# balisujohn/tortoise.cpp

Hardware: AMD Instinct MI355X
Metric: audio-seconds/sec end-to-end (AR+diffusion+vocoder), 16 cands x 80 steps (higher is better)
Workload: dtype f16 MFMA inputs / f32 accumulate (diffusion, vocoder convs); f32 weights, f16 KV (AR)

## Files before the change

### tortoise.cpp_amd/csrc/gemm_f16.h

```cpp
#pragma once
#include <hip/hip_fp16.h>
#include <hip/hip_runtime.h>
#include <algorithm>
#include <cmath>
#include <cstdlib>
#include <type_traits>

namespace tts {

typedef _Float16 half8 __attribute__((ext_vector_type(8)));
typedef float floatx4 __attribute__((ext_vector_type(4)));

enum { GEMM_OUT_F32 = 0, GEMM_OUT_F16 = 1, GEMM_OUT_QKV = 2, GEMM_OUT_QKV_SPLIT = 3, GEMM_OUT_F32_SCALED = 4, GEMM_OUT_F32_STATS = 5, GEMM_OUT_F32_SCALED_STATS = 6 };
constexpr bool gemm_mode_qkv(int mode) { return mode == GEMM_OUT_QKV || mode == GEMM_OUT_QKV_SPLIT; }
constexpr bool gemm_mode_f32(int mode) { return mode == GEMM_OUT_F32 || mode == GEMM_OUT_F32_SCALED || mode == GEMM_OUT_F32_STATS || mode == GEMM_OUT_F32_SCALED_STATS; }
constexpr bool gemm_mode_scaled(int mode) { return mode == GEMM_OUT_F32_SCALED || mode == GEMM_OUT_F32_SCALED_STATS; }
constexpr bool gemm_mode_stats(int mode) { return mode == GEMM_OUT_F32_STATS || mode == GEMM_OUT_F32_SCALED_STATS; }

struct GemmArgs {
  const __half *A[3];
  int row_off[3];
  int nseg, kseg;
  int lda;
  const __half *W;
  int ldw_, w_off_[3], custom_w;
  const __half *Wf;
  int wreg;
  int M, N;
  const float *bias;
  const int *row_seq;
  float *outF; int ldo; const float *resid;
  __half *outH; int ldh;
  __half *outVt; int ldvt;
  __half *outH2, *outVt2;
  float alpha;
  long long *st_out;
  int st_stripe_ll;
  const int *chunk_seq;
  int dual_b;
  int mode;
  int th, cn;
  int ku;
};


__device__ __forceinline__ int lds_swz(int row) { return ((row >> 1) & 3) << 1; }
__device__ __forceinline__ int lds_off(int row, int chunk) { return row * 128 + ((chunk ^ lds_swz(row)) << 4); }

typedef const void __attribute__((address_space(1))) *gptr_t;
typedef void __attribute__((address_space(3))) *lptr_t;

__device__ __forceinline__ int vh_blk(int wm, int i) { return wm + 2 * i; }

__device__ __forceinline__ float split_lo(float x) { return x - __half2float(__float2half_rn(x)); }
__device__ __forceinline__ uint2 pack_half4(float a, float b, float c, float d) {
  const __half2 p0 = __floats2half2_rn(a, b), p1 = __floats2half2_rn(c, d);
  uint2 u;
  u.x = *(const unsigned *)&p0;
  u.y = *(const unsigned *)&p1;
  return u;
}

static constexpr int FX_STRIPES = 8;
__device__ __forceinline__ void fx_add(long long *dst, float p) {
  const float h = rintf(p * 256.0f);
  const float rem = p - h * (1.0f / 256.0f);
  atomicAdd((unsigned long long *)dst, (unsigned long long)(long long)h);
  atomicAdd((unsigned long long *)dst + 1, (unsigned long long)(long long)rintf(rem * 4503599627370496.0f));
}
__device__ __forceinline__ void fx_split(float p, long long &hi, long long &lo) {
  const float h = rintf(p * 256.0f);
  hi = (long long)h;
  lo = (long long)rintf((p - h * (1.0f / 256.0f)) * 4503599627370496.0f);
}
__host__ __device__ __forceinline__ double fx_value(long long hi, long long lo) { return (double)hi * (1.0 / 256.0) + (double)lo * (1.0 / 1152921504606846976.0); }
template <int CTRL> __device__ __forceinline__ float gemm_dpp(float x) {
  return __int_as_float(__builtin_amdgcn_update_dpp(0, __float_as_int(x), CTRL, 0xf, 0xf, false));
}
__device__ __forceinline__ float red_half_block(float x) {
  x += gemm_dpp<0xB1>(x);
  x += gemm_dpp<0x4E>(x);
  x += gemm_dpp<0x141>(x);
  auto a = __builtin_amdgcn_permlane32_swap(__float_as_uint(x), __float_as_uint(x), false, false);
  x = __uint_as_float(a[0]) + __uint_as_float(a[1]);
  auto b = __builtin_amdgcn_permlane16_swap(__float_as_uint(x), __float_as_uint(x), false, false);
  return __uint_as_float(b[0]) + __uint_as_float(b[1]);
}

enum { EPI_NO_RESID = 0, EPI_RESID_IN_ACC = 1, EPI_RESID_LOAD = 2 };
template <int MODE, int MI, int RESID>
__device__ __forceinline__ void gemm_epilogue_vh(const GemmArgs &g, floatx4 (&acc)[MI > 0 ? MI : 1][4], int m0, int n0, int wm, int wn, int fr, int fq) {
  constexpr int MA = MI > 0 ? MI : 1;
  if (MI == 0) return;
  if (gemm_mode_qkv(MODE)) {
    const int c0 = n0 + wn * 64, h = c0 / 192, w0 = c0 - h * 192;
    if (w0 >= 128) {
      const bool hb = g.bias != nullptr, hs = g.row_seq != nullptr;
      const float *bp = hb ? g.bias : (const float *)g.W;
      const int *sp = hs ? g.row_seq : (const int *)g.A[0];
      float bv[4];
      int4 sq[MA];
#pragma unroll
      for (int j = 0; j < 4; j++) bv[j] = bp[c0 + j * 16 + fr];
#pragma unroll
      for (int i = 0; i < MI; i++) sq[i] = *(const int4 *)(sp + m0 + vh_blk(wm, i) * 16 + fq * 4);
#pragma unroll
      for (int j = 0; j < 4; j++) bv[j] = hb ? bv[j] : 0.f;
#pragma unroll
      for (int i = 0; i < MI; i++) sq[i] = hs ? sq[i] : make_int4(0, 0, 0, 0);
#pragma unroll
      for (int i = 0; i < MI; i++) {
        const int rbase = m0 + vh_blk(wm, i) * 16 + fq * 4;
        const bool gd[4] = {sq[i].x < 0, sq[i].y < 0, sq[i].z < 0, sq[i].w < 0};
#pragma unroll
        for (int j = 0; j < 4; j++) {
          float v[4];
#pragma unroll
          for (int r = 0; r < 4; r++) v[r] = gd[r] ? 0.f : acc[i][j][r] + bv[j];
          *(uint2 *)(g.outVt + (size_t)(h * 64 + j * 16 + fr) * g.ldvt + rbase) = pack_half4(v[0], v[1], v[2], v[3]);
          if (MODE == GEMM_OUT_QKV_SPLIT)
            *(uint2 *)(g.outVt2 + (size_t)(h * 64 + j * 16 + fr) * g.ldvt + rbase) = pack_half4(split_lo(v[0]), split_lo(v[1]), split_lo(v[2]), split_lo(v[3]));
        }
      }
      return;
    }
  }
  const int col0 = n0 + wn * 64 + fq * 4;
  const bool hb = g.bias != nullptr, hs = g.row_seq != nullptr;
  const float *bp = hb ? g.bias : (const float *)g.W;
  const int *sp = hs ? g.row_seq : (const int *)g.A[0];
  float4 b4[4];
  int sq[MA];
  float4 rr[2][4];
  auto load_pair = [&](int p) {
#pragma unroll
    for (int q = 0; q < 2; q++) {
      const int i = min(2 * p + q, MI - 1);
      const float *rp = g.resid + (size_t)(m0 + vh_blk(wm, i) * 16 + fr) * g.ldo + col0;
#pragma unroll
      for (int j = 0; j < 4; j++) rr[q][j] = *(const float4 *)(rp + j * 16);
    }
  };
  if (RESID == EPI_RESID_LOAD) load_pair(0);
#pragma unroll
  for (int j = 0; j < 4; j++) b4[j] = *(const float4 *)(bp + col0 + j * 16);
#pragma unroll
  for (int i = 0; i < MI; i++) sq[i] = sp[m0 + vh_blk(wm, i) * 16 + fr];
#pragma unroll
  for (int j = 0; j < 4; j++) b4[j] = hb ? b4[j] : make_float4(0.f, 0.f, 0.f, 0.f);
#pragma unroll
  for (int i = 0; i < MI; i++) sq[i] = hs ? sq[i] : 0;
  auto finish = [&](int i, int j) {
    if (gemm_mode_scaled(MODE)) acc[i][j] *= g.alpha;
    float4 v = make_float4(acc[i][j][0] + b4[j].x, acc[i][j][1] + b4[j].y, acc[i][j][2] + b4[j].z, acc[i][j][3] + b4[j].w);
    if (sq[i] < 0) v = make_float4(0.f, 0.f, 0.f, 0.f);
    return v;
  };
  if (gemm_mode_f32(MODE)) {
    float ssum[MA][2], ssq[MA][2];
// ... 363 lines not shown
  int sq[MI];
#pragma unroll
  for (int j = 0; j < 2; j++) b4[j] = *(const float4 *)(bp + col0 + j * 16);
#pragma unroll
  for (int i = 0; i < MI; i++) sq[i] = sp[m0 + min(i, nblk - 1) * 16 + fr];
#pragma unroll
  for (int j = 0; j < 2; j++) b4[j] = hb ? b4[j] : make_float4(0.f, 0.f, 0.f, 0.f);
#pragma unroll
  for (int i = 0; i < MI; i++) sq[i] = hs ? sq[i] : 0;
  auto finish = [&](int i, int j) {
    float4 v = make_float4(acc[i][j][0] + b4[j].x, acc[i][j][1] + b4[j].y, acc[i][j][2] + b4[j].z, acc[i][j][3] + b4[j].w);
    if (sq[i] < 0) v = make_float4(0.f, 0.f, 0.f, 0.f);
    return v;
  };
  if (MODE == GEMM_OUT_F32) {
#pragma unroll
    for (int i = 0; i < MI; i++) {
      if (i < nblk) {
        float *op = g.outF + (size_t)(m0 + i * 16 + fr) * g.ldo + col0;
#pragma unroll
        for (int j = 0; j < 2; j++) *(float4 *)(op + j * 16) = finish(i, j);
      }
    }
  } else {
    const int h = c0 / 192, w0 = c0 - h * 192;
#pragma unroll
    for (int i = 0; i < MI; i++) {
      if (i < nblk) {
        __half *op = g.outH + (size_t)(m0 + i * 16 + fr) * g.ldh + h * 128 + w0 + fq * 4;
#pragma unroll
        for (int j = 0; j < 2; j++) {
          const float4 v = finish(i, j);
          *(uint2 *)(op + j * 16) = pack_half4(v.x, v.y, v.z, v.w);
          if (MODE == GEMM_OUT_QKV_SPLIT)
            *(uint2 *)(g.outH2 + (op - g.outH) + j * 16) = pack_half4(split_lo(v.x), split_lo(v.y), split_lo(v.z), split_lo(v.w));
        }
      }
    }
  }
}

template <int MODE, int MI, int D, bool NAT>
__device__ __forceinline__ void gemm_wreg_body(const GemmArgs &g, int m0, int n0, int nblk, int lane, int wave) {
  extern __shared__ __attribute__((aligned(16))) char smem_dyn[];
  char *smem = smem_dyn;
  constexpr int S = D + 1;
  constexpr int NPA = MI / 2;
  constexpr int PER = NPA + 4;
  static_assert(D == 1 || D == 2, "prefetch distance");
  const int T = g.kseg >> 6, KS = g.kseg >> 5;
  const int fr = lane & 15, fq = lane >> 4;
  unsigned aoff[NPA];
#pragma unroll
  for (int i = 0; i < NPA; i++) aoff[i] = (unsigned)(gemm_dma_off(wave + 4 * i, lane, 0, nblk * 16 - 1, g.lda) * 2);
  const char *aseg = (const char *)(g.A[0] + (ptrdiff_t)(g.row_off[0] + m0) * g.lda);
  const __half *wp0 = g.Wf + (size_t)((n0 >> 4) + wave * 2) * KS * 512, *wp1 = wp0 + (size_t)KS * 512;
  const unsigned wlane = lane * 16;
  const bool resid_first = MODE == GEMM_OUT_F32 && g.resid != nullptr;
  floatx4 acc[MI][2];
  gemm_acc_start<MODE, MI, 2>(g, acc, resid_first, n0 + wave * 32, fq, [&](int i) { return m0 + min(i, nblk - 1) * 16 + fr; });
  half8 w[S][2][2];
  auto issue = [&](int t, auto set_c) {
    constexpr int U = decltype(set_c)::value;
    const char *ab = aseg + (t << 7);
#pragma unroll
    for (int i = 0; i < NPA; i++) __builtin_amdgcn_global_load_lds((gptr_t)(ab + aoff[i]), (lptr_t)(smem + U * 16384 + (wave + 4 * i) * 1024), 16, 0, 0);
    const __half *q0 = wp0 + (size_t)t * 1024, *q1 = wp1 + (size_t)t * 1024;
    wreg_load<0>(w[U][0][0], q0, wlane);
    wreg_load<0>(w[U][0][1], q1, wlane);
    wreg_load<1024>(w[U][1][0], q0, wlane);
    wreg_load<1024>(w[U][1][1], q1, wlane);
  };
  auto kloop = [&]() {
    auto step = [&](int t, auto u_c) {
      constexpr int U = decltype(u_c)::value;
      if (D == 2 && t + 1 < T) wreg_wait<PER>(w[U][0][0], w[U][0][1], w[U][1][0], w[U][1][1]);
      else wreg_wait<0>(w[U][0][0], w[U][0][1], w[U][1][0], w[U][1][1]);
      asm volatile("s_waitcnt lgkmcnt(0)" ::: "memory");
      __builtin_amdgcn_s_barrier();
      if (t + D < T) issue(t + D, std::integral_constant<int, (U + D) % S>{});
      const char *sa = smem + U * 16384;
      constexpr int AHEAD = 2;
      half8 af[AHEAD + 1];
      auto frag = [&](int x) { return *(const half8 *)(sa + lds_off((x % MI) * 16 + fr, (x / MI) * 4 + fq)); };
#pragma unroll
      for (int x = 0; x < AHEAD; x++) af[x] = frag(x);
#pragma unroll
      for (int x = 0; x < 2 * MI; x++) {
        if (x + AHEAD < 2 * MI) af[(x + AHEAD) % (AHEAD + 1)] = frag(x + AHEAD);
        const int ks = x / MI, i = x % MI;
        const half8 a = af[x % (AHEAD + 1)];
#pragma unroll
        for (int j = 0; j < 2; j++) {
          if (NAT) acc[i][j] = __builtin_amdgcn_mfma_f32_16x16x32_f16(a, w[U][ks][j], acc[i][j], 0, 0, 0);
          else acc[i][j] = __builtin_amdgcn_mfma_f32_16x16x32_f16(w[U][ks][j], a, acc[i][j], 0, 0, 0);
        }
      }
      __builtin_amdgcn_sched_group_barrier(0x100, AHEAD, 0);
#pragma unroll
      for (int x = 0; x < 2 * MI; x++) {
        if (x + AHEAD < 2 * MI) __builtin_amdgcn_sched_group_barrier(0x100, 1, 0);
        __builtin_amdgcn_sched_group_barrier(0x008, 2, 0);
      }
    };
    for (int t0 = 0; t0 < T; t0 += S) {
      step(t0, std::integral_constant<int, 0>{});
      if (t0 + 1 < T) step(t0 + 1, std::integral_constant<int, 1>{});
      if (S == 3 && t0 + 2 < T) step(t0 + 2, std::integral_constant<int, S - 1>{});
    }
  };
  issue(0, std::integral_constant<int, 0>{});
  if (D == 2) issue(1, std::integral_constant<int, 1>{});
#pragma unroll
  for (int i = 0; i < MI; i++)
#pragma unroll
    for (int j = 0; j < 2; j++) asm volatile("" : "+v"(acc[i][j]));
  kloop();
  gemm_epilogue_wreg<MODE, MI, NAT>(g, acc, m0, n0, nblk, wave, fr, fq);
}

static constexpr int GEMM_WREG_D = 1, GEMM_WREG_LDS = (GEMM_WREG_D + 1) * 16384;
template <int MODE, int D = GEMM_WREG_D>
static __global__ __launch_bounds__(256, 4) void gemm_f16_wreg_kernel(GemmArgs g) {
  const int tid = threadIdx.x, lane = tid & 63, wave = __builtin_amdgcn_readfirstlane(tid >> 6);
  int m0, n0, nblk;
  if (!gemm_vh_tile(g, m0, n0, nblk)) return;
  if (gemm_mode_qkv(MODE) && ((n0 + wave * 32) % 192) >= 128) {
    if (nblk > 4) gemm_wreg_body<MODE, 8, D, true>(g, m0, n0, nblk, lane, wave);
    else gemm_wreg_body<MODE, 4, D, true>(g, m0, n0, nblk, lane, wave);
  } else {
    if (nblk > 4) gemm_wreg_body<MODE, 8, D, false>(g, m0, n0, nblk, lane, wave);
    else gemm_wreg_body<MODE, 4, D, false>(g, m0, n0, nblk, lane, wave);
  }
}
static inline bool gemm_takes_wreg(const GemmArgs &g, int th, int ku) {
  return g.wreg > 0 && g.Wf && g.nseg == 1 && !g.custom_w && th == 8 && ku == 1 && (g.kseg >> 6) >= 2 &&
         (g.mode == GEMM_OUT_F32 || g.mode == GEMM_OUT_QKV || g.mode == GEMM_OUT_QKV_SPLIT);
}

struct GemmGnPanelArgs {
  const __half *A; int lda;
  const __half *Wf;
  int N, K;
  const float *bias;
  const int *seq_start, *seq_len; int ns, rows_total;
  float eps; const float *gn_g, *gn_b, *ss; int do_silu, lut; __half *y; const int *seq_step; int ss_step_stride;
};
static constexpr int GEMM_GN_PANEL_ROWS = 896, GEMM_GN_PANEL_LDS = GEMM_GN_PANEL_ROWS * 128;
static constexpr int GEMM_GN_PANEL_WRING = 2 * 8192, GEMM_GN_PANEL_LDS_LAUNCH = GEMM_GN_PANEL_LDS + GEMM_GN_PANEL_WRING;
__device__ __forceinline__ int gnp_panel_f4(int t, int q) { return t * 128 + ((q ^ (t & 7)) << 4); }
template <int OFF> __device__ __forceinline__ void gnp_lds_read(half8 &d, unsigned addr) {
  asm volatile("ds_read_b128 %0, %1 offset:%2" : "=v"(d) : "v"(addr), "i"(OFF));
}
static inline int gemm_auto_th(int M, int N);
static inline bool gemm_gn_panel_takes(int option, bool stats, bool debug_sums, bool has_wf, int max_len, int rows, int N, int K) {
  return option != 0 && !stats && !debug_sums && has_wf && max_len >= 1 && max_len <= GEMM_GN_PANEL_ROWS && gemm_auto_th(rows, N) == 8 && (N % 64) == 0 && K >= 64 && (K % 64) == 0;
}
static inline int gemm_gn_panel_grid(int ns, int N) { return 8 * ((ns * (N >> 6) + 7) / 8); }

template <class TAIL>
static __global__ __launch_bounds__(512) void gemm_f16_gn_panel_kernel(GemmGnPanelArgs a, TAIL tail) {
  extern __shared__ __attribute__((aligned(16))) char smem_dyn[];
  char *smem = smem_dyn;
  const int tid = threadIdx.x, lane = tid & 63, wave = __builtin_amdgcn_readfirstlane(tid >> 6);
  const int np = a.N >> 6, nitems = a.ns * np, xcd = blockIdx.x & 7, idx = blockIdx.x >> 3;
  const int i0 = (int)((long long)nitems * xcd >> 3), i1 = (int)((long long)nitems * (xcd + 1) >> 3);
  if (idx >= i1 - i0) return;
  const int item = i0 + idx, s = item / np, n0 = (item - s * np) << 6;
  const int T = a.seq_len[s], r0 = a.seq_start[s];
  const int KT = a.K >> 6, fr = lane & 15, fq = lane >> 4;
  const int rb = wave * 112 + (lane >> 3), lda2 = a.lda * 2;
  const unsigned coloff = (unsigned)(((lane & 7) ^ lds_swz(lane >> 3)) << 4);
  const char *aseg = (const char *)(a.A + (size_t)r0 * a.lda);
  const size_t wstride = (size_t)(a.K >> 5) * 512;
  const __half *wsrc = a.Wf + (size_t)((n0 >> 4) + (wave & 3)) * wstride + (wave >> 2) * 512 + lane * 8;
  char *wring = smem + GEMM_GN_PANEL_LDS;
  const unsigned wfb = (unsigned)(size_t)(lptr_t)wring + lane * 16;
  const unsigned lds0 = (unsigned)(size_t)(lptr_t)smem + wave * 7 * 2048;
  const unsigned fb0 = lds0 + lds_off(fr, fq), fb1 = lds0 + lds_off(fr, 4 + fq);
  floatx4 acc[7][4];
#pragma unroll
  for (int i = 0; i < 7; i++)
#pragma unroll
    for (int j = 0; j < 4; j++) acc[i][j] = (floatx4){0.f, 0.f, 0.f, 0.f};
  auto dma = [&](int t) {
    const char *ab = aseg + (t << 7);
    int rbv = rb;
    asm volatile("" : "+v"(rbv));
#pragma unroll
    for (int i = 0; i < 14; i++) {
      const unsigned off = (unsigned)(min(rbv + 8 * i, T - 1) * lda2) + coloff;
      __builtin_amdgcn_global_load_lds((gptr_t)(ab + off), (lptr_t)(smem + (wave * 14 + i) * 1024), 16, 0, 0);
    }
  };
  auto wdma = [&](int t) { __builtin_amdgcn_global_load_lds((gptr_t)(wsrc + (size_t)t * 1024), (lptr_t)(wring + ((t & 1) << 13) + wave * 1024), 16, 0, 0); };
  auto step = [&](int t, auto last_c) {
    constexpr bool LAST = decltype(last_c)::value;
    asm volatile("s_waitcnt vmcnt(1)" ::: "memory");
    half8 af[2][7], w[2][4];
    gnp_lds_read<0 * 2048>(af[0][0], fb0);
    gnp_lds_read<1 * 2048>(af[0][1], fb0);
    gnp_lds_read<2 * 2048>(af[0][2], fb0);
    gnp_lds_read<3 * 2048>(af[0][3], fb0);
    gnp_lds_read<4 * 2048>(af[0][4], fb0);
    gnp_lds_read<5 * 2048>(af[0][5], fb0);
    gnp_lds_read<6 * 2048>(af[0][6], fb0);
    gnp_lds_read<0 * 2048>(af[1][0], fb1);
    gnp_lds_read<1 * 2048>(af[1][1], fb1);
    gnp_lds_read<2 * 2048>(af[1][2], fb1);
    gnp_lds_read<3 * 2048>(af[1][3], fb1);
    gnp_lds_read<4 * 2048>(af[1][4], fb1);
    gnp_lds_read<5 * 2048>(af[1][5], fb1);
    gnp_lds_read<6 * 2048>(af[1][6], fb1);
    asm volatile("s_waitcnt lgkmcnt(0)"
                 : "+v"(af[0][0]), "+v"(af[0][1]), "+v"(af[0][2]), "+v"(af[0][3]), "+v"(af[0][4]), "+v"(af[0][5]), "+v"(af[0][6]), "+v"(af[1][0]), "+v"(af[1][1]),
                   "+v"(af[1][2]), "+v"(af[1][3]), "+v"(af[1][4]), "+v"(af[1][5]), "+v"(af[1][6])
                 :
                 : "memory");
    if (!LAST) dma(t + 1);
    if (LAST) asm volatile("s_waitcnt vmcnt(0)" ::: "memory");
    else asm volatile("s_waitcnt vmcnt(14)" ::: "memory");
    __builtin_amdgcn_s_barrier();
    asm volatile("" ::: "memory");
    if (!LAST) wdma(t + 1);
    const unsigned wf = wfb + ((t & 1) << 13);
    gnp_lds_read<0 * 1024>(w[0][0], wf);
    gnp_lds_read<1 * 1024>(w[0][1], wf);
    gnp_lds_read<2 * 1024>(w[0][2], wf);
    gnp_lds_read<3 * 1024>(w[0][3], wf);
    gnp_lds_read<4 * 1024>(w[1][0], wf);
    gnp_lds_read<5 * 1024>(w[1][1], wf);
    gnp_lds_read<6 * 1024>(w[1][2], wf);
    gnp_lds_read<7 * 1024>(w[1][3], wf);
    asm volatile("s_waitcnt lgkmcnt(0)" : "+v"(w[0][0]), "+v"(w[0][1]), "+v"(w[0][2]), "+v"(w[0][3]), "+v"(w[1][0]), "+v"(w[1][1]), "+v"(w[1][2]), "+v"(w[1][3]) : : "memory");
    __builtin_amdgcn_sched_barrier(0);
#pragma unroll
    for (int ks = 0; ks < 2; ks++)
#pragma unroll
      for (int i = 0; i < 7; i++)
#pragma unroll
        for (int j = 0; j < 4; j++) acc[i][j] = __builtin_amdgcn_mfma_f32_16x16x32_f16(w[ks][j], af[ks][i], acc[i][j], 0, 0, 0);
  };
  dma(0);
  wdma(0);
  for (int t = 0; t + 1 < KT; t++) step(t, std::false_type{});
  step(KT - 1, std::true_type{});
  const bool hb = a.bias != nullptr;
  const float *bp = hb ? a.bias : (const float *)a.Wf;
  float4 b4[4];
#pragma unroll
  for (int j = 0; j < 4; j++) b4[j] = *(const float4 *)(bp + n0 + j * 16 + fq * 4);
#pragma unroll
  for (int j = 0; j < 4; j++) b4[j] = hb ? b4[j] : make_float4(0.f, 0.f, 0.f, 0.f);
#pragma unroll
  for (int gi = 0; gi < 2; gi++) {
#pragma unroll
    for (int i = 0; i < 7; i++) {
      const int row = (wave * 7 + i) * 16 + fr;
#pragma unroll
      for (int jj = 0; jj < 2; jj++) {
        const int j = gi * 2 + jj;
        *(float4 *)(smem + gnp_panel_f4(row, jj * 4 + fq)) = make_float4(acc[i][j][0] + b4[j].x, acc[i][j][1] + b4[j].y, acc[i][j][2] + b4[j].z, acc[i][j][3] + b4[j].w);
      }
    }
    __syncthreads();
    tail(a, s, T, r0, n0 + gi * 32, smem);
  }
}

static constexpr int CONV3_VH_LDS = (128 + 8) * 128 + 2 * 16384;
template <int MODE, int MI>
__device__ __forceinline__ void gemm_conv3_vh_body(const GemmArgs &g, int m0, int n0, int nblk, int lane, int wave) {
  extern __shared__ __attribute__((aligned(16))) char smem_dyn[];
  char *smem = smem_dyn;
  constexpr int MA = MI > 0 ? MI : 1;
  const int wm = wave >> 1, wn = wave & 1;
  const int my_pa = (2 * nblk + 1 - wave + 3) >> 2;
  const int nchunks = g.kseg >> 6, ldw = 3 * g.kseg, nph = 3 * nchunks;
  const int prow = lane >> 3, pslot = lane & 7;
  const int fr = lane & 15, fq = lane >> 4;
  floatx4 acc[MA][4];
#pragma unroll
  for (int i = 0; i < MI; i++)
#pragma unroll
    for (int j = 0; j < 4; j++) acc[i][j] = (floatx4){0.f, 0.f, 0.f, 0.f};
  char *sa = smem, *sb = smem + (128 + 8) * 128;
  const __half *abase = g.A[0] + (ptrdiff_t)(m0 - 1) * g.lda;
  const __half *wbase = g.W + (size_t)n0 * ldw;
  int aoff[5], boff[4];
#pragma unroll
  for (int i = 0; i < 5; i++) {
    const int row = (wave + 4 * i) * 8 + prow;
    aoff[i] = min(row, g.M - m0 + 1) * g.lda + (pslot ^ lds_swz(row)) * 8;
  }
#pragma unroll
  for (int i = 0; i < 4; i++) {
    const int row = (wave * 4 + i) * 8 + prow;
    boff[i] = row * ldw + (pslot ^ lds_swz(row)) * 8;
  }
  auto stageA = [&](int kc) {
    const __half *src = abase + (min(kc, nchunks - 1) << 6);
#pragma unroll
    for (int i = 0; i < 5; i++)
      if (i < my_pa) __builtin_amdgcn_global_load_lds((gptr_t)(src + aoff[i]), (lptr_t)(sa + (wave + 4 * i) * 1024), 16, 0, 0);
  };
  auto stageB = [&](int p) {
    p = min(p, nph - 1);
    const int kc = p / 3, tap = p - kc * 3;
    const __half *src = wbase + tap * g.kseg + (kc << 6);
    char *dst = sb + (p & 1) * 16384;
#pragma unroll
    for (int i = 0; i < 4; i++) __builtin_amdgcn_global_load_lds((gptr_t)(src + boff[i]), (lptr_t)(dst + (wave * 4 + i) * 1024), 16, 0, 0);
  };
  auto phase = [&](int kc, int p, auto tap_c) {
    constexpr int TAP = decltype(tap_c)::value;
    stageB(p + 1);
    asm volatile("s_waitcnt vmcnt(4)" ::: "memory");
    __builtin_amdgcn_s_barrier();
    const char *sbp = sb + (p & 1) * 16384;
#pragma unroll
    for (int ks = 0; ks < 2; ks++) {
      half8 af[MA], bf[4];
#pragma unroll
      for (int i = 0; i < MI; i++) af[i] = *(const half8 *)(sa + lds_off(vh_blk(wm, i) * 16 + fr + TAP, ks * 4 + fq));
      if (MI > 0) {
#pragma unroll
        for (int i = 0; i < 4; i++) bf[i] = *(const half8 *)(sbp + lds_off(wn * 64 + i * 16 + fr, ks * 4 + fq));
      }
#pragma unroll
      for (int i = 0; i < MI; i++)
#pragma unroll
        for (int j = 0; j < 4; j++) acc[i][j] = __builtin_amdgcn_mfma_f32_16x16x32_f16(bf[j], af[i], acc[i][j], 0, 0, 0);
    }
    asm volatile("s_waitcnt lgkmcnt(0)" ::: "memory");
    __builtin_amdgcn_s_barrier();
    if (TAP == 2) stageA(kc + 1);
  };
  stageA(0);
  stageB(0);
  for (int kc = 0; kc < nchunks; kc++) {
    const int p = 3 * kc;
    phase(kc, p, std::integral_constant<int, 0>{});
    phase(kc, p + 1, std::integral_constant<int, 1>{});
    phase(kc, p + 2, std::integral_constant<int, 2>{});
  }
  asm volatile("s_waitcnt vmcnt(0)" ::: "memory");
  if ((MODE == GEMM_OUT_F32 || MODE == GEMM_OUT_F32_STATS) && g.resid) gemm_epilogue_vh<MODE, MI, EPI_RESID_LOAD>(g, acc, m0, n0, wm, wn, fr, fq);
  else gemm_epilogue_vh<MODE, MI, EPI_NO_RESID>(g, acc, m0, n0, wm, wn, fr, fq);
}

template <int MODE>
static __global__ __launch_bounds__(256, 3) void gemm_f16_conv3_vh_kernel(GemmArgs g) {
  const int tid = threadIdx.x, lane = tid & 63, wave = __builtin_amdgcn_readfirstlane(tid >> 6);
  int m0, n0, nblk;
  if (!gemm_vh_tile(g, m0, n0, nblk)) return;
  gemm_for_my_mi(nblk, wave, [&](auto mi) { gemm_conv3_vh_body<MODE, decltype(mi)::value>(g, m0, n0, nblk, lane, wave); });
}

static inline bool gemm_is_conv3(const GemmArgs &g) {
  return g.nseg == 3 && !g.custom_w && g.A[0] == g.A[1] && g.A[1] == g.A[2] && g.row_off[0] == -1 && g.row_off[1] == 0 && g.row_off[2] == 1 &&
         !gemm_mode_qkv(g.mode) && !gemm_mode_scaled(g.mode);
}

static inline size_t gemm_wfrag3_index(int n, int tap, int k, int N, int K) {
  return (size_t)tap * N * K + gemm_wfrag_index(n, k, K);
}
static constexpr int CONV3_WREG_SLOT = (128 + 8) * 128, CONV3_WREG_LDS = 2 * CONV3_WREG_SLOT;

template <int MI, bool RESID>
__device__ __forceinline__ void gemm_epilogue_conv3_wreg(const GemmArgs &g, floatx4 (&acc)[MI][2], int m0, int n0, int nblk, int wave, int fr, int fq) {
  const int col0 = n0 + wave * 32 + fq * 4;
  const bool hb = g.bias != nullptr, hs = g.row_seq != nullptr;
  const float *bp = hb ? g.bias : (const float *)g.W;
  const int *sp = hs ? g.row_seq : (const int *)g.A[0];
  float4 b4[2], rr[2][2];
  int sq[MI];
  auto load_pair = [&](int p) {
#pragma unroll
    for (int q = 0; q < 2; q++) {
      const float *rp = g.resid + (size_t)(m0 + min(2 * p + q, nblk - 1) * 16 + fr) * g.ldo + col0;
#pragma unroll
      for (int j = 0; j < 2; j++) rr[q][j] = *(const float4 *)(rp + j * 16);
    }
  };
  if (RESID) load_pair(0);
#pragma unroll
  for (int j = 0; j < 2; j++) b4[j] = *(const float4 *)(bp + col0 + j * 16);
#pragma unroll
  for (int i = 0; i < MI; i++) sq[i] = sp[m0 + min(i, nblk - 1) * 16 + fr];
#pragma unroll
  for (int j = 0; j < 2; j++) b4[j] = hb ? b4[j] : make_float4(0.f, 0.f, 0.f, 0.f);
#pragma unroll
  for (int i = 0; i < MI; i++) sq[i] = hs ? sq[i] : 0;
#pragma unroll
  for (int p = 0; p < MI / 2; p++) {
    float4 v[2][2];
#pragma unroll
// ... 233 lines not shown
```

### tortoise.cpp_amd/testlib/gemm_gn_panel_harness.hip

```cpp
#include "../csrc/diffusion.hip"

#include <cstdint>
#include <cstring>
#include <vector>

using namespace tts;
hipEvent_t tts::prof_event(tts_ctx *) { return nullptr; }

extern "C" {

enum { TTS_GNP_TEST_MARGIN = 4096, TTS_GNP_TEST_SENTINEL = 0xCB, TTS_GNP_TEST_MAX_SEQ = 64, TTS_GNP_TEST_MAX_ROWS = 8192, TTS_GNP_TEST_MAX_TABLE = 64,
       TTS_GNP_TEST_MAX_STRIDE = 1 << 16 };

struct tts_gnp_case {
  int ns, rows, N, K;
  int do_silu, lut, n_steps, ss_step_stride;
  float eps;
  const int *start, *len, *seq_step;
  const uint16_t *A, *W;
  const float *bias, *g, *b, *ss;
  void *out_pair, *out_fused;
};

int tts_gnp_test_margin(void) { return TTS_GNP_TEST_MARGIN; }
int tts_gnp_test_takes(int option, int stats, int debug_sums, int has_wf, int max_len, int rows, int N, int K) {
  return gemm_gn_panel_takes(option, stats != 0, debug_sums != 0, has_wf != 0, max_len, rows, N, K) ? 1 : 0;
}
int tts_gnp_test_grid(int ns, int N) { return gemm_gn_panel_grid(ns, N); }
int tts_gnp_test_lds(void) { return GEMM_GN_PANEL_LDS; }

}

namespace {

struct Dev {
  char *p = nullptr;
  size_t bytes = 0;
  ~Dev() { if (p) (void)hipFree(p); }
  hipError_t alloc(size_t payload, int fill) {
    bytes = payload;
    hipError_t e = hipMalloc((void **)&p, payload + 2 * TTS_GNP_TEST_MARGIN);
    if (e != hipSuccess) { p = nullptr; return e; }
    return hipMemset(p, fill, payload + 2 * TTS_GNP_TEST_MARGIN);
  }
  char *data() const { return p ? p + TTS_GNP_TEST_MARGIN : nullptr; }
  hipError_t put(const void *h) { return hipMemcpy(data(), h, bytes, hipMemcpyHostToDevice); }
  hipError_t get_all(void *h) const { return hipMemcpy(h, p, bytes + 2 * TTS_GNP_TEST_MARGIN, hipMemcpyDeviceToHost); }
};

int nw_of(int N) { return (N + 127) / 128 * 128; }

bool valid(const tts_gnp_case &c) {
  if (!c.A || !c.W || !c.g || !c.b || !c.out_pair || !c.out_fused || !c.start || !c.len) return false;
  if (c.rows < 128 || c.rows % 128 || c.rows > TTS_GNP_TEST_MAX_ROWS) return false;
  if (c.N < 64 || c.N % 64 || c.N > C || c.K < 128 || c.K % 64 || c.K > 2048) return false;
  if (c.ns < 1 || c.ns > TTS_GNP_TEST_MAX_SEQ) return false;
  long long prev_end = 0;
  for (int s = 0; s < c.ns; s++) {
    const long long st = c.start[s], ln = c.len[s];
    if (st < prev_end || st % 8 || ln < 1 || ln > GEMM_GN_PANEL_ROWS || st + ln + 1 > c.rows) return false;
    prev_end = st + ln + 1;
  }
  if (c.lut < 0 || c.lut > 2 || (c.do_silu != 0 && c.do_silu != 1)) return false;
  if (c.seq_step && !c.ss) return false;
  if (c.ss) {
    if (c.n_steps < 1 || c.n_steps > TTS_GNP_TEST_MAX_TABLE || c.ss_step_stride < 0 || c.ss_step_stride > TTS_GNP_TEST_MAX_STRIDE) return false;
    if (!c.seq_step && c.n_steps != 1) return false;
    if (c.seq_step)
      for (int s = 0; s < c.ns; s++)
        if (c.seq_step[s] < 0 || c.seq_step[s] >= c.n_steps) return false;
  }
  return true;
}

}

extern "C" {

int tts_gnp_test_validate(const tts_gnp_case *c) { return c && valid(*c) ? 0 : (int)hipErrorInvalidValue; }

#define HT(x) do { hipError_t e_ = (x); if (e_ != hipSuccess) return (int)e_; } while (0)

int tts_gnp_test_run(const tts_gnp_case *cp) {
  if (!cp || !valid(*cp)) return (int)hipErrorInvalidValue;
  const tts_gnp_case &c = *cp;
  const int rows = c.rows, Nw = nw_of(c.N), K = c.K;
  GemmArgs g{};
  for (int i = 0; i < 3; i++) { g.A[i] = nullptr; g.row_off[i] = 0; }
  g.nseg = 1; g.kseg = K; g.lda = K; g.M = rows; g.N = Nw; g.mode = GEMM_OUT_F32; g.ldo = C; g.wreg = 1; g.th = 8;
  g.Wf = (const __half *)c.W;
  if (gemm_plan(g).err != hipSuccess || gemm_plan(g).kernel != GEMM_KERNEL_WREG) return (int)hipErrorInvalidValue;

  std::vector<uint16_t> wf((size_t)Nw * K);
  for (int n = 0; n < Nw; n++)
    for (int k = 0; k < K; k++) wf[gemm_wfrag_index(n, k, K)] = c.W[(size_t)n * K + k];
  std::vector<int> rs(rows, -1);
  for (int s = 0; s < c.ns; s++)
    for (int t = 0; t < c.len[s]; t++) rs[c.start[s] + t] = s;

  Dev A, W, Wf, bias, gg, bb, ss, step, start, len, rseq, H, yp, yf;
  HT(A.alloc((size_t)rows * K * 2, 0)); HT(A.put(c.A));
  HT(W.alloc((size_t)Nw * K * 2, 0)); HT(W.put(c.W));
  HT(Wf.alloc((size_t)Nw * K * 2, 0)); HT(Wf.put(wf.data()));
  if (c.bias) { HT(bias.alloc((size_t)Nw * 4, 0)); HT(bias.put(c.bias)); }
  HT(gg.alloc((size_t)C * 4, 0)); HT(gg.put(c.g));
  HT(bb.alloc((size_t)C * 4, 0)); HT(bb.put(c.b));
  if (c.ss) {
    HT(ss.alloc(((size_t)(c.n_steps - 1) * c.ss_step_stride + 2 * C) * 4, 0)); HT(ss.put(c.ss));
    if (c.seq_step) { HT(step.alloc((size_t)c.ns * 4, 0)); HT(step.put(c.seq_step)); }
  }
  HT(start.alloc((size_t)c.ns * 4, 0)); HT(start.put(c.start));
  HT(len.alloc((size_t)c.ns * 4, 0)); HT(len.put(c.len));
  HT(rseq.alloc((size_t)rows * 4, 0)); HT(rseq.put(rs.data()));
  HT(H.alloc((size_t)rows * C * 4, 0));
  HT(yp.alloc((size_t)rows * C * 2, TTS_GNP_TEST_SENTINEL));
  HT(yf.alloc((size_t)rows * C * 2, TTS_GNP_TEST_SENTINEL));

  for (int i = 0; i < 3; i++) g.A[i] = (const __half *)A.data();
  g.W = (const __half *)W.data(); g.Wf = (const __half *)Wf.data(); g.bias = (const float *)bias.data();
  g.row_seq = (const int *)rseq.data(); g.outF = (float *)H.data(); g.resid = nullptr;
  const int *d_start = (const int *)start.data(), *d_len = (const int *)len.data(), *d_step = (const int *)step.data();
  GemmGnPanelArgs a{};
  a.A = (const __half *)A.data(); a.lda = K; a.Wf = (const __half *)Wf.data(); a.N = c.N; a.K = K; a.bias = (const float *)bias.data();
  a.seq_start = d_start; a.seq_len = d_len; a.ns = c.ns; a.rows_total = rows;
  a.eps = c.eps; a.gn_g = (const float *)gg.data(); a.gn_b = (const float *)bb.data(); a.ss = (const float *)ss.data(); a.do_silu = c.do_silu; a.lut = c.lut;
  a.y = (__half *)yf.data(); a.seq_step = d_step; a.ss_step_stride = c.ss_step_stride;

  hipStream_t s;
  HT(hipStreamCreateWithFlags(&s, hipStreamNonBlocking));
  hipError_t e = hipDeviceSynchronize();
  if (e == hipSuccess) e = launch_gemm_f16(g, s);
  if (e == hipSuccess) {
    gn_reg_kernel<512, 14><<<dim3(32, c.ns), 512, 0, s>>>((const float *)H.data(), d_start, d_len, rows, c.ns, c.eps, a.gn_g, a.gn_b, a.ss, c.do_silu, c.lut,
                                                          (__half *)yp.data(), nullptr, 0, nullptr, 0, d_step, c.ss_step_stride);
    e = hipGetLastError();
  }
  if (e == hipSuccess) e = launch_gemm_gn_panel(a, s);
  const hipError_t es = hipStreamSynchronize(s);
  (void)hipStreamDestroy(s);
  if (e != hipSuccess || es != hipSuccess) return (int)(e != hipSuccess ? e : es);
  HT(yp.get_all(c.out_pair));
  HT(yf.get_all(c.out_fused));
  return 0;
}

}
```

Baseline: 140.0.

## Interleave A-panel DMA and LDS fragment reads with MFMA blocks in GN panel GEMM

Restructures the GN-panel GEMM inner step so the next tile's A-panel global-to-LDS loads are issued in seven chunks interleaved with the seven MFMA row blocks. A-fragment LDS reads are also software-pipelined one block ahead, replacing the up-front load-all-then-compute pattern. Fine-grained vmcnt waits track the split DMA. The goal is to hide global and LDS latency behind MFMA work, at the cost of more complex waitcnt accounting that must stay correct. The test harness also relaxes K to allow 64.

```diff
diff --git a/tortoise.cpp_amd/csrc/gemm_f16.h b/tortoise.cpp_amd/csrc/gemm_f16.h
--- a/tortoise.cpp_amd/csrc/gemm_f16.h
+++ b/tortoise.cpp_amd/csrc/gemm_f16.h
@@ -5,6 +5,7 @@
 #include <cmath>
 #include <cstdlib>
 #include <type_traits>
+#include <utility>
 
 namespace tts {
 
@@ -674,6 +675,9 @@
 template <int OFF> __device__ __forceinline__ void gnp_lds_read(half8 &d, unsigned addr) {
   asm volatile("ds_read_b128 %0, %1 offset:%2" : "=v"(d) : "v"(addr), "i"(OFF));
 }
+template <int N> __device__ __forceinline__ void gnp_vm_wait() { asm volatile("s_waitcnt vmcnt(%0)" : : "i"(N) : "memory"); }
+template <class F, int... I> __device__ __forceinline__ void gnp_for_blocks_seq(F &&f, std::integer_sequence<int, I...>) { (f(std::integral_constant<int, I>{}), ...); }
+template <class F> __device__ __forceinline__ void gnp_for_blocks(F &&f) { gnp_for_blocks_seq(f, std::make_integer_sequence<int, 7>{}); }
 static inline int gemm_auto_th(int M, int N);
 static inline bool gemm_gn_panel_takes(int option, bool stats, bool debug_sums, bool has_wf, int max_len, int rows, int N, int K) {
   return option != 0 && !stats && !debug_sums && has_wf && max_len >= 1 && max_len <= GEMM_GN_PANEL_ROWS && gemm_auto_th(rows, N) == 8 && (N % 64) == 0 && K >= 64 && (K % 64) == 0;
@@ -705,43 +709,21 @@
   for (int i = 0; i < 7; i++)
 #pragma unroll
     for (int j = 0; j < 4; j++) acc[i][j] = (floatx4){0.f, 0.f, 0.f, 0.f};
-  auto dma = [&](int t) {
+  auto dma2 = [&](int t, int i, int rbv) {
     const char *ab = aseg + (t << 7);
-    int rbv = rb;
-    asm volatile("" : "+v"(rbv));
-#pragma unroll
-    for (int i = 0; i < 14; i++) {
-      const unsigned off = (unsigned)(min(rbv + 8 * i, T - 1) * lda2) + coloff;
-      __builtin_amdgcn_global_load_lds((gptr_t)(ab + off), (lptr_t)(smem + (wave * 14 + i) * 1024), 16, 0, 0);
+#pragma unroll
+    for (int h = 0; h < 2; h++) {
+      const unsigned off = (unsigned)(min(rbv + 16 * i + 8 * h, T - 1) * lda2) + coloff;
+      __builtin_amdgcn_global_load_lds((gptr_t)(ab + off), (lptr_t)(smem + (wave * 14 + 2 * i + h) * 1024), 16, 0, 0);
     }
   };
   auto wdma = [&](int t) { __builtin_amdgcn_global_load_lds((gptr_t)(wsrc + (size_t)t * 1024), (lptr_t)(wring + ((t & 1) << 13) + wave * 1024), 16, 0, 0); };
   auto step = [&](int t, auto last_c) {
     constexpr bool LAST = decltype(last_c)::value;
-    asm volatile("s_waitcnt vmcnt(1)" ::: "memory");
+    int rbv = rb;
+    asm volatile("" : "+v"(rbv));
     half8 af[2][7], w[2][4];
-    gnp_lds_read<0 * 2048>(af[0][0], fb0);
-    gnp_lds_read<1 * 2048>(af[0][1], fb0);
-    gnp_lds_read<2 * 2048>(af[0][2], fb0);
-    gnp_lds_read<3 * 2048>(af[0][3], fb0);
-    gnp_lds_read<4 * 2048>(af[0][4], fb0);
-    gnp_lds_read<5 * 2048>(af[0][5], fb0);
-    gnp_lds_read<6 * 2048>(af[0][6], fb0);
-    gnp_lds_read<0 * 2048>(af[1][0], fb1);
-    gnp_lds_read<1 * 2048>(af[1][1], fb1);
-    gnp_lds_read<2 * 2048>(af[1][2], fb1);
-    gnp_lds_read<3 * 2048>(af[1][3], fb1);
-    gnp_lds_read<4 * 2048>(af[1][4], fb1);
-    gnp_lds_read<5 * 2048>(af[1][5], fb1);
-    gnp_lds_read<6 * 2048>(af[1][6], fb1);
-    asm volatile("s_waitcnt lgkmcnt(0)"
-                 : "+v"(af[0][0]), "+v"(af[0][1]), "+v"(af[0][2]), "+v"(af[0][3]), "+v"(af[0][4]), "+v"(af[0][5]), "+v"(af[0][6]), "+v"(af[1][0]), "+v"(af[1][1]),
-                   "+v"(af[1][2]), "+v"(af[1][3]), "+v"(af[1][4]), "+v"(af[1][5]), "+v"(af[1][6])
-                 :
-                 : "memory");
-    if (!LAST) dma(t + 1);
-    if (LAST) asm volatile("s_waitcnt vmcnt(0)" ::: "memory");
-    else asm volatile("s_waitcnt vmcnt(14)" ::: "memory");
+    asm volatile("s_waitcnt vmcnt(14)" ::: "memory");
     __builtin_amdgcn_s_barrier();
     asm volatile("" ::: "memory");
     if (!LAST) wdma(t + 1);
@@ -754,17 +736,40 @@
     gnp_lds_read<5 * 1024>(w[1][1], wf);
     gnp_lds_read<6 * 1024>(w[1][2], wf);
     gnp_lds_read<7 * 1024>(w[1][3], wf);
-    asm volatile("s_waitcnt lgkmcnt(0)" : "+v"(w[0][0]), "+v"(w[0][1]), "+v"(w[0][2]), "+v"(w[0][3]), "+v"(w[1][0]), "+v"(w[1][1]), "+v"(w[1][2]), "+v"(w[1][3]) : : "memory");
+    if (LAST) asm volatile("s_waitcnt vmcnt(12)" ::: "memory");
+    else asm volatile("s_waitcnt vmcnt(13)" ::: "memory");
+    gnp_lds_read<0>(af[0][0], fb0);
+    gnp_lds_read<0>(af[1][0], fb1);
+    asm volatile("s_waitcnt lgkmcnt(0)"
+                 : "+v"(w[0][0]), "+v"(w[0][1]), "+v"(w[0][2]), "+v"(w[0][3]), "+v"(w[1][0]), "+v"(w[1][1]), "+v"(w[1][2]), "+v"(w[1][3]), "+v"(af[0][0]), "+v"(af[1][0])
+                 :
+                 : "memory");
     __builtin_amdgcn_sched_barrier(0);
-#pragma unroll
-    for (int ks = 0; ks < 2; ks++)
-#pragma unroll
-      for (int i = 0; i < 7; i++)
+    gnp_for_blocks([&](auto i_c) {
+      constexpr int i = decltype(i_c)::value, n = i < 6 ? i + 1 : 6;
+      if constexpr (i < 6) {
+        gnp_vm_wait<LAST ? 10 - 2 * i : 11>();
+        gnp_lds_read<n * 2048>(af[0][n], fb0);
+        gnp_lds_read<n * 2048>(af[1][n], fb1);
+      }
+      if (!LAST) dma2(t + 1, i, rbv);
+      __builtin_amdgcn_sched_barrier(0);
+#pragma unroll
+      for (int ks = 0; ks < 2; ks++)
 #pragma unroll
         for (int j = 0; j < 4; j++) acc[i][j] = __builtin_amdgcn_mfma_f32_16x16x32_f16(w[ks][j], af[ks][i], acc[i][j], 0, 0, 0);
-  };
-  dma(0);
-  wdma(0);
+      __builtin_amdgcn_sched_barrier(0);
+      if constexpr (i < 6) asm volatile("s_waitcnt lgkmcnt(0)" : "+v"(af[0][n]), "+v"(af[1][n]) : : "memory");
+      __builtin_amdgcn_sched_barrier(0);
+    });
+  };
+  {
+    int rbv = rb;
+    asm volatile("" : "+v"(rbv));
+    wdma(0);
+#pragma unroll
+    for (int i = 0; i < 7; i++) dma2(0, i, rbv);
+  }
   for (int t = 0; t + 1 < KT; t++) step(t, std::false_type{});
   step(KT - 1, std::true_type{});
   const bool hb = a.bias != nullptr;
diff --git a/tortoise.cpp_amd/testlib/gemm_gn_panel_harness.hip b/tortoise.cpp_amd/testlib/gemm_gn_panel_harness.hip
--- a/tortoise.cpp_amd/testlib/gemm_gn_panel_harness.hip
+++ b/tortoise.cpp_amd/testlib/gemm_gn_panel_harness.hip
@@ -53,7 +53,7 @@
 bool valid(const tts_gnp_case &c) {
   if (!c.A || !c.W || !c.g || !c.b || !c.out_pair || !c.out_fused || !c.start || !c.len) return false;
   if (c.rows < 128 || c.rows % 128 || c.rows > TTS_GNP_TEST_MAX_ROWS) return false;
-  if (c.N < 64 || c.N % 64 || c.N > C || c.K < 128 || c.K % 64 || c.K > 2048) return false;
+  if (c.N < 64 || c.N % 64 || c.N > C || c.K < 64 || c.K % 64 || c.K > 2048) return false;
   if (c.ns < 1 || c.ns > TTS_GNP_TEST_MAX_SEQ) return false;
   long long prev_end = 0;
   for (int s = 0; s < c.ns; s++) {
@@ -89,7 +89,7 @@
   for (int i = 0; i < 3; i++) { g.A[i] = nullptr; g.row_off[i] = 0; }
   g.nseg = 1; g.kseg = K; g.lda = K; g.M = rows; g.N = Nw; g.mode = GEMM_OUT_F32; g.ldo = C; g.wreg = 1; g.th = 8;
   g.Wf = (const __half *)c.W;
-  if (gemm_plan(g).err != hipSuccess || gemm_plan(g).kernel != GEMM_KERNEL_WREG) return (int)hipErrorInvalidValue;
+  if (gemm_plan(g).err != hipSuccess || gemm_plan(g).kernel != (K >= 128 ? GEMM_KERNEL_WREG : GEMM_KERNEL_VH)) return (int)hipErrorInvalidValue;
 
   std::vector<uint16_t> wf((size_t)Nw * K);
   for (int n = 0; n < Nw; n++)
```

Result: no change. 140.2 (median of 3 runs) (+0.2%).
